# achiever04/face-recognition-platform

Measured on AMD Instinct MI355X. Metric: faces/sec (detect+embed+match) on 1080p @ 100k gallery, higher is better.
Workload: dtype f16; 1 GPU; 32x1080x1920 BGR frames per GPU per step resident in HBM, host results out every step, 2 batches in flight per GPU (one handle = one stream each, used round-robin), forced K=10 faces/frame, 100000-identity fp16 gallery, FRPDet detector fp16 + ArcFace IResNet-100 fp16 (synthetic seeded weights); batch_frames=32, faces_per_frame=10, gallery=100000, streams=1, lanes=2, lane_warmup_steps=20

## Files before the change

### face-recognition-platform_amd/csrc/decode_nms.hip

```cpp
#include <hip/hip_runtime.h>
#include <stdint.h>
#include "frp_internal.h"

namespace frp {

#define NMS_CAP 1024
#define NT 1024

__device__ __forceinline__ unsigned sortable16(unsigned short h) {
    if ((h & 0x7fffu) > 0x7c00u) return 0u;
    return (h & 0x8000u) ? (unsigned)(unsigned short)(~h) : (unsigned)(h | 0x8000u);
}
__device__ __forceinline__ bool is_candidate(_Float16 lg, float lt) {
    return lt == -INFINITY ? true : (float)lg >= lt;
}

struct FrameView {
    const _Float16 *h0, *h1, *h2;
    int w0, w1, w2;
    int e0, e1;
};

__device__ __forceinline__ const _Float16* anchor_ptr(const FrameView& fv, int idx, int& level, int& x, int& y) {
    level = idx < fv.e0 ? 0 : (idx < fv.e1 ? 1 : 2);
    const int li = idx - (level == 0 ? 0 : (level == 1 ? fv.e0 : fv.e1));
    const int wl = level == 0 ? fv.w0 : (level == 1 ? fv.w1 : fv.w2);
    const _Float16* base = level == 0 ? fv.h0 : (level == 1 ? fv.h1 : fv.h2);
    const int pos = li >> 1, a = li & 1;
    y = pos / wl;
    x = pos - y * wl;
    return base + (long)pos * 32 + a * 15;
}

__device__ __forceinline__ FrameView frame_view(const DecodeParams& p, int b, int& A) {
    FrameView fv;
    fv.h0 = p.head[0] + (long)b * p.hl[0] * p.wl[0] * 32;
    fv.h1 = p.head[1] + (long)b * p.hl[1] * p.wl[1] * 32;
    fv.h2 = p.head[2] + (long)b * p.hl[2] * p.wl[2] * 32;
    fv.w0 = p.wl[0]; fv.w1 = p.wl[1]; fv.w2 = p.wl[2];
    fv.e0 = p.hl[0] * p.wl[0] * 2;
    fv.e1 = fv.e0 + p.hl[1] * p.wl[1] * 2;
    A = fv.e1 + p.hl[2] * p.wl[2] * 2;
    return fv;
}

__global__ __launch_bounds__(256) void gather_logits_kernel(DecodeParams p) {
    int A;
    const FrameView fv = frame_view(p, blockIdx.y, A);
    const int i = blockIdx.x * 256 + threadIdx.x;
    if (i >= A) return;
    int lv, x, y;
    p.logits[(long)blockIdx.y * A + i] = anchor_ptr(fv, i, lv, x, y)[0];
}

__global__ __launch_bounds__(NT) void decode_nms_kernel(DecodeParams p) {
    __shared__ unsigned long long keys[NMS_CAP];
    __shared__ int hist[4096];
    __shared__ float bx1[NMS_CAP], by1[NMS_CAP], bx2[NMS_CAP], by2[NMS_CAP], barea[NMS_CAP];
    __shared__ unsigned char supp[NMS_CAP];
    __shared__ int s_cnt, s_digit, s_need, s_keepn;
    __shared__ int s_keep[FRP_MAX_FACES_CAP];
    __shared__ int wsum[NT / 64];

    const int b = blockIdx.x;
    const int tid = threadIdx.x;
    int A;
    const FrameView fv = frame_view(p, b, A);
    const float lt = p.logit_thresh;

    if (tid == 0) { s_cnt = 0; s_keepn = 0; }
    __syncthreads();
    const _Float16* dense = p.logits + (long)b * A;
    int local = 0;
    for (int i = tid; i < A; i += NT) local += is_candidate(dense[i], lt) ? 1 : 0;
#pragma unroll
    for (int o = 32; o > 0; o >>= 1) local += __shfl_xor(local, o);
    if ((tid & 63) == 0) atomicAdd(&s_cnt, local);
    __syncthreads();
    const int total = s_cnt;
    __syncthreads();

    unsigned long long T = 0ull;
    if (total > NMS_CAP) {
        unsigned long long prefix = 0ull;
        int need = NMS_CAP;
        for (int pass = 0; pass < 3; ++pass) {
            const int shift = 24 - 12 * pass;
            for (int i = tid; i < 4096; i += NT) hist[i] = 0;
            __syncthreads();
            for (int i = tid; i < A; i += NT) {
                const _Float16 lg = dense[i];
                if (is_candidate(lg, lt)) {
                    const unsigned long long k = ((unsigned long long)sortable16(__builtin_bit_cast(unsigned short, lg)) << 20) |
                                                 (unsigned long long)(0xFFFFF - i);
                    if (pass == 0 || (k >> (shift + 12)) == prefix) atomicAdd(&hist[(int)((k >> shift) & 0xFFF)], 1);
                }
            }
            __syncthreads();
            const int b0 = tid * 4;
            const int h0 = hist[b0], h1 = hist[b0 + 1], h2 = hist[b0 + 2], h3 = hist[b0 + 3];
            const int mine = h0 + h1 + h2 + h3;
            int v = mine;
#pragma unroll
            for (int o = 1; o < 64; o <<= 1) {
                const int n = __shfl_down(v, o);
                if ((tid & 63) + o < 64) v += n;
            }
            if ((tid & 63) == 0) wsum[tid >> 6] = v;
            __syncthreads();
            int above_waves = 0;
            for (int w = (tid >> 6) + 1; w < NT / 64; ++w) above_waves += wsum[w];
            const int suffix_incl = v + above_waves;
            const int above = suffix_incl - mine;
            int c = above;
            if (c < need && need <= c + h3) { s_digit = b0 + 3; s_need = need - c; }
            c += h3;
            if (c < need && need <= c + h2) { s_digit = b0 + 2; s_need = need - c; }
            c += h2;
            if (c < need && need <= c + h1) { s_digit = b0 + 1; s_need = need - c; }
            c += h1;
            if (c < need && need <= c + h0) { s_digit = b0; s_need = need - c; }
            __syncthreads();
            prefix = (prefix << 12) | (unsigned long long)s_digit;
            need = s_need;
            __syncthreads();
        }
        T = prefix;
    }

    if (tid == 0) s_cnt = 0;
    for (int i = tid; i < NMS_CAP; i += NT) { keys[i] = 0ull; supp[i] = 0; }
    __syncthreads();
    for (int i = tid; i < A; i += NT) {
        const _Float16 lg = dense[i];
        if (is_candidate(lg, lt)) {
            const unsigned long long k = ((unsigned long long)sortable16(__builtin_bit_cast(unsigned short, lg)) << 20) |
                                         (unsigned long long)(0xFFFFF - i);
            if (k >= T) {
                const int s = atomicAdd(&s_cnt, 1);
                if (s < NMS_CAP) keys[s] = k | (1ull << 40);
            }
        }
    }
    __syncthreads();
    const int n = s_cnt < NMS_CAP ? s_cnt : NMS_CAP;

    for (int k2 = 2; k2 <= NMS_CAP; k2 <<= 1) {
        for (int j = k2 >> 1; j > 0; j >>= 1) {
            const int i = tid;
            const int ixj = i ^ j;
            if (ixj > i) {
                const unsigned long long a = keys[i], c = keys[ixj];
                const bool desc = (i & k2) == 0;
                if (desc ? (a < c) : (a > c)) { keys[i] = c; keys[ixj] = a; }
            }
            __syncthreads();
        }
    }

    if (tid < n) {
        const int idx = 0xFFFFF - (int)(keys[tid] & 0xFFFFF);
        int lv, x, y;
        const _Float16* q = anchor_ptr(fv, idx, lv, x, y);
        const float s = (float)(8 << lv);
        const float cx = (float)(x * (8 << lv)), cy = (float)(y * (8 << lv));
        const float x1 = cx - (float)q[1] * s, y1 = cy - (float)q[2] * s;
        const float x2 = cx + (float)q[3] * s, y2 = cy + (float)q[4] * s;
        bx1[tid] = x1; by1[tid] = y1; bx2[tid] = x2; by2[tid] = y2;
        barea[tid] = (x2 - x1 + 1.0f) * (y2 - y1 + 1.0f);
    }
    __syncthreads();

    const int K = p.max_faces;
    for (int i = 0; i < n; ++i) {
        if (supp[i]) continue;
        if (tid == 0) s_keep[s_keepn] = i;
        const int kept = s_keepn + 1;
        if (kept >= K) { __syncthreads(); if (tid == 0) s_keepn = kept; __syncthreads(); break; }
        const float ix1 = bx1[i], iy1 = by1[i], ix2 = bx2[i], iy2 = by2[i], ia = barea[i];
        for (int j = i + 1 + tid; j < n; j += NT) {
            const float xx1 = fmaxf(ix1, bx1[j]), yy1 = fmaxf(iy1, by1[j]);
            const float xx2 = fminf(ix2, bx2[j]), yy2 = fminf(iy2, by2[j]);
            const float w = fmaxf(0.0f, xx2 - xx1 + 1.0f), h = fmaxf(0.0f, yy2 - yy1 + 1.0f);
            const float inter = w * h;
            const float ovr = inter / ((ia + barea[j]) - inter);
            if (ovr > p.nms_iou) supp[j] = 1;
        }
        __syncthreads();
        if (tid == 0) s_keepn = kept;
        __syncthreads();
    }
    __syncthreads();
    const int kept = s_keepn;

    if (tid < K) {
        float* ob = p.boxes + ((long)b * K + tid) * 4;
        float* ok = p.kps + ((long)b * K + tid) * 10;
        if (tid < kept) {
            const int c = s_keep[tid];
            const int idx = 0xFFFFF - (int)(keys[c] & 0xFFFFF);
            int lv, x, y;
            const _Float16* q = anchor_ptr(fv, idx, lv, x, y);
            const float s = (float)(8 << lv);
            const float cx = (float)(x * (8 << lv)), cy = (float)(y * (8 << lv));
            ob[0] = bx1[c]; ob[1] = by1[c]; ob[2] = bx2[c]; ob[3] = by2[c];
#pragma unroll
            for (int t = 0; t < 5; ++t) {
                ok[2 * t] = cx + (float)q[5 + 2 * t] * s;
                ok[2 * t + 1] = cy + (float)q[6 + 2 * t] * s;
            }
            p.scores[(long)b * K + tid] = 1.0f / (1.0f + expf(-(float)q[0]));
            if (p.anchor) p.anchor[(long)b * K + tid] = idx;
        } else {
            ob[0] = ob[1] = ob[2] = ob[3] = 0.f;
            for (int t = 0; t < 10; ++t) ok[t] = 0.f;
            p.scores[(long)b * K + tid] = 0.f;
            if (p.anchor) p.anchor[(long)b * K + tid] = -1;
        }
    }
    if (tid == 0) p.counts[b] = kept;
}

__global__ __launch_bounds__(256) void resize_u8_kernel(const uint8_t* __restrict__ src, int B, int H, int W,
                                                        uint8_t* __restrict__ dst, int Hs, int Ws, float ry, float rx) {
    const long total = (long)B * Hs * Ws;
    for (long i = (long)blockIdx.x * blockDim.x + threadIdx.x; i < total; i += (long)gridDim.x * blockDim.x) {
        const int x = (int)(i % Ws);
        const long r = i / Ws;
        const int y = (int)(r % Hs);
        const int b = (int)(r / Hs);
        float sy = ((float)y + 0.5f) * ry - 0.5f, sx = ((float)x + 0.5f) * rx - 0.5f;
        sy = fminf(fmaxf(sy, 0.0f), (float)(H - 1));
        sx = fminf(fmaxf(sx, 0.0f), (float)(W - 1));
        const int y0 = (int)sy, x0 = (int)sx;
        const int y1 = y0 + 1 < H ? y0 + 1 : H - 1, x1 = x0 + 1 < W ? x0 + 1 : W - 1;
        const float fy = sy - (float)y0, fx = sx - (float)x0;
        const uint8_t* p00 = src + (((long)b * H + y0) * W + x0) * 3;
        const uint8_t* p01 = src + (((long)b * H + y0) * W + x1) * 3;
        const uint8_t* p10 = src + (((long)b * H + y1) * W + x0) * 3;
        const uint8_t* p11 = src + (((long)b * H + y1) * W + x1) * 3;
        uint8_t* o = dst + i * 3;
#pragma unroll
        for (int c = 0; c < 3; ++c) {
            const float top = (float)p00[c] * (1.0f - fx) + (float)p01[c] * fx;
            const float bot = (float)p10[c] * (1.0f - fx) + (float)p11[c] * fx;
            const float v = top * (1.0f - fy) + bot * fy;
            o[c] = (uint8_t)fminf(fmaxf(floorf(v + 0.5f), 0.0f), 255.0f);
        }
    }
}

hipError_t launch_resize_u8(const uint8_t* src, int B, int H, int W, uint8_t* dst, int Hs, int Ws, hipStream_t stream) {
    if (!src || !dst || B <= 0 || H <= 0 || W <= 0 || Hs <= 0 || Ws <= 0) return hipErrorInvalidValue;
    const long total = (long)B * Hs * Ws;
    const int grid = (int)((total + 255) / 256 < 16384 ? (total + 255) / 256 : 16384);
    hipLaunchKernelGGL(resize_u8_kernel, dim3(grid), dim3(256), 0, stream, src, B, H, W, dst, Hs, Ws,
                       (float)H / (float)Hs, (float)W / (float)Ws);
    return hipGetLastError();
}

hipError_t launch_decode_nms(const DecodeParams& p, hipStream_t stream) {
    if (p.B <= 0 || p.max_faces <= 0 || p.max_faces > FRP_MAX_FACES_CAP) return hipErrorInvalidValue;
    long A = 0;
    for (int l = 0; l < 3; ++l) {
        if (!p.head[l] || p.hl[l] <= 0 || p.wl[l] <= 0) return hipErrorInvalidValue;
        A += (long)p.hl[l] * p.wl[l] * 2;
    }
    if (A > 0xFFFFF) return hipErrorInvalidValue;
    if (!p.boxes || !p.kps || !p.scores || !p.counts || !p.logits) return hipErrorInvalidValue;
    hipLaunchKernelGGL(gather_logits_kernel, dim3((unsigned)((A + 255) / 256), p.B), dim3(256), 0, stream, p);
    hipError_t e = hipGetLastError();
    if (e != hipSuccess) return e;
    hipLaunchKernelGGL(decode_nms_kernel, dim3(p.B), dim3(NT), 0, stream, p);
    return hipGetLastError();
}

}
```

### face-recognition-platform_amd/csrc/frp_api.cpp

```cpp
#include <hip/hip_runtime.h>

#include <algorithm>
#include <cmath>
#include <cstdio>
#include <cstdlib>
#include <cstring>
#include <mutex>
#include <string>
#include <vector>

#include "frp.h"
#include "frp_blob.h"
#include "frp_internal.h"
#include "frp_handle.h"

using namespace frp;

#define FRP_WINO_MIN_FACES 128
Switches frp::read_switches() {
    auto set = [](const char* n) { return getenv(n) ? 1 : 0; };
    const char *sm = getenv("FRP_SMALL_M"), *wm = getenv("FRP_WINO_MIN_FACES");
    Switches s{};
    s.small_m = !sm ? 0 : (sm[0] == '0' ? -1 : 1);
    s.wino_min_faces = wm ? atoi(wm) : FRP_WINO_MIN_FACES;
    s.s2 = set("FRP_S2"); s.host_count = set("FRP_HOST_COUNT"); s.match_v1 = set("FRP_MATCH_V1");
    s.no_fused_stem12 = set("FRP_NO_FUSED_STEM12"); s.no_fused_stem = set("FRP_NO_FUSED_STEM");
    s.no_emb_stem = set("FRP_NO_EMB_STEM"); s.no_stem_fuse = set("FRP_NO_STEM_FUSE");
    s.no_wino = set("FRP_NO_WINO"); s.no_kconcat = set("FRP_NO_KCONCAT");
    s.no_block_fuse = set("FRP_NO_BLOCK_FUSE"); s.block_fuse_all = set("FRP_BLOCK_FUSE_ALL");
    return s;
}

const ProcessSwitches& frp::process_switches() {
    static const ProcessSwitches s = [] {
        const char* jh = getenv("FRP_JPEG_DEVICE_HUFFMAN");
        const char* js = getenv("FRP_JPEG_SELFSYNC");
        return ProcessSwitches{getenv("FRP_NO_GRAPH") != nullptr, getenv("FRP_C64_ALL") != nullptr, !jh ? 0 : (jh[0] == '0' ? -1 : 1), js && js[0] != '0'};
    }();
    return s;
}

namespace {

float logit_threshold(float t) {
    if (!(t > 0.f)) return -INFINITY;
    if (t >= 1.f) return INFINITY;
    return (float)std::log((double)t / (1.0 - (double)t));
}

bool det_size_ok(int Hs, int Ws) { return Hs > 0 && Ws > 0 && Hs <= 16384 && Ws <= 16384; }

int select_det_source(frp_handle* h, int Hs, int Ws) {
    if (h->rB <= 0) return fail(h, FRP_ERR_INVALID, "no resident frames (call frp_upload_frames)");
    if (!det_size_ok(Hs, Ws)) return fail(h, FRP_ERR_INVALID, "bad detector size");
    if (Hs == h->rH && Ws == h->rW) {
        h->det_scaled = false;
    } else {
        FRPCHK(ensure(h, h->scaled, (size_t)h->rB * Hs * Ws * 3));
        hipError_t e = launch_resize_u8((const uint8_t*)h->frames.p, h->rB, h->rH, h->rW, (uint8_t*)h->scaled.p, Hs, Ws, h->stream);
        if (e != hipSuccess) return fail(h, FRP_ERR_HIP, std::string("resize: ") + hipGetErrorString(e));
        h->det_scaled = true;
    }
    h->dH = Hs; h->dW = Ws;
    h->canvas_h = round_up(Hs, 32);
    h->canvas_w = round_up(Ws, 32);
    return FRP_OK;
}

int ensure_results(frp_handle* h, int B, int K) {
    const size_t s = (size_t)B * K;
    FRPCHK(ensure(h, h->boxes, s * 4 * 4));
    FRPCHK(ensure(h, h->kps, s * 10 * 4));
    FRPCHK(ensure(h, h->scores, s * 4));
    FRPCHK(ensure(h, h->anchor, s * 4));
    FRPCHK(ensure(h, h->counts, (size_t)B * 4));
    FRPCHK(ensure(h, h->face_slot, s * 4));
    FRPCHK(ensure(h, h->nfaces, 16));
    return FRP_OK;
}

struct DetOut {
    float *boxes, *kps, *scores;
    int32_t* counts;
};

int run_decode(frp_handle* h, const void* const head[3], const int dims[3][2], int B, int K, float det_thresh, float nms_iou, uint32_t flags,
               const DetOut* out = nullptr) {
    DecodeParams dp{};
    size_t anchors = 0;
    for (int l = 0; l < 3; ++l) {
        dp.head[l] = (const _Float16*)head[l];
        dp.hl[l] = dims[l][0];
        dp.wl[l] = dims[l][1];
        anchors += (size_t)dp.hl[l] * dp.wl[l] * 2;
    }
    dp.B = B;
    dp.max_faces = K;
    const bool forced = flags & FRP_FLAG_FORCED_K;
    dp.logit_thresh = forced ? -INFINITY : logit_threshold(det_thresh);
    dp.nms_iou = forced ? 2.0f : nms_iou;
    if (out) {
        dp.boxes = out->boxes; dp.kps = out->kps; dp.scores = out->scores; dp.counts = out->counts;
    } else {
        dp.boxes = (float*)h->boxes.p; dp.kps = (float*)h->kps.p; dp.scores = (float*)h->scores.p;
        dp.anchor = (int32_t*)h->anchor.p; dp.counts = (int32_t*)h->counts.p;
    }
    FRPCHK(ensure(h, h->dense_logits, (size_t)B * anchors * 2));
    dp.logits = (_Float16*)h->dense_logits.p;
    const hipError_t e = launch_decode_nms(dp, h->stream);
    if (e != hipSuccess) return fail(h, FRP_ERR_HIP, std::string("decode_nms: ") + hipGetErrorString(e));
    return FRP_OK;
}

int compact_faces(frp_handle* h, int B, int K) {
    hipError_t e = launch_compact_faces((const int32_t*)h->counts.p, B, K, (int32_t*)h->face_slot.p, (int32_t*)h->nfaces.p, h->stream);
    if (e != hipSuccess) return fail(h, FRP_ERR_HIP, std::string("compact_faces: ") + hipGetErrorString(e));
    return FRP_OK;
}

StemParams stem_params(const frp_handle* h, uint32_t flags) {
    StemParams sp{};
    sp.frames = h->det_scaled ? (const uint8_t*)h->scaled.p : (const uint8_t*)h->frames.p;
    sp.B = h->rB; sp.H = h->dH; sp.W = h->dW;
    sp.row_stride = (long)h->dW * 3; sp.frame_stride = (long)h->dH * h->dW * 3;
    sp.Hc = h->canvas_h; sp.Wc = h->canvas_w; sp.Ho = sp.Hc / 2; sp.Wo = sp.Wc / 2;
    sp.rgb_in = (flags & FRP_FLAG_RGB) ? 1 : 0;
    return sp;
}

bool det_wino(const frp_handle* h) {
    return (long)h->rB * (h->canvas_h / 8) * (h->canvas_w / 8) >= 2L * 240 * (h->n_cu > 0 ? h->n_cu : 256);
}

int run_detect(frp_handle* h, const Switches& sw, int K, float det_thresh, float nms_iou, uint32_t flags, const DetOut* out = nullptr) {
    if (!h->have_weights) return fail(h, FRP_ERR_NO_WEIGHTS, "no weights loaded");
    if (h->rB <= 0) return fail(h, FRP_ERR_INVALID, "no resident frames (call frp_upload_frames)");
    if (K <= 0 || K > FRP_MAX_FACES_CAP) return fail(h, FRP_ERR_INVALID, "max_faces out of range");
    const int B = h->rB, Hc = h->canvas_h, Wc = h->canvas_w;
    const bool fused = h->det.det_stem && !sw.no_fused_stem;
    FRPCHK(plan_net(h, h->det, B, Hc, Wc, fused));
    if (!out) FRPCHK(ensure_results(h, B, K));
    const StemParams sp = stem_params(h, flags);
    if (!fused) {
        hipError_t e = launch_preprocess(sp.frames, B, sp.H, sp.W, sp.row_stride, sp.frame_stride, (_Float16*)h->det.bufs[h->det.in_buf].p, Hc, Wc,
                                         sp.rgb_in, h->stream);
        if (e != hipSuccess) return fail(h, FRP_ERR_HIP, std::string("preprocess: ") + hipGetErrorString(e));
    }
    rec(h, EV_PRE);
    FRPCHK(run_net(h, sw, h->det, B, Hc, Wc, &h->ctr.det_conv_flops, &h->ctr.det_conv_launches, fused ? &sp : nullptr, nullptr, det_wino(h)));
    rec(h, EV_DET);
    const void* head[3];
    int dims[3][2];
    for (int l = 0; l < 3; ++l) {
        const int bi = (int)h->hdr.det_head_buf[l];
        head[l] = h->det.bufs[bi].p;
        dims[l][0] = h->det.dims[bi].h;
        dims[l][1] = h->det.dims[bi].w;
        if (h->det.dims[bi].c != 32) return fail(h, FRP_ERR_BLOB, "detector head must have 32 channels");
    }
    FRPCHK(run_decode(h, head, dims, B, K, det_thresh, nms_iou, flags, out));
    if (!out && !(flags & FRP_FLAG_TRACK)) FRPCHK(compact_faces(h, B, K));
    rec(h, EV_DEC);
    return FRP_OK;
}

int run_embed(frp_handle* h, const Switches& sw, int n, const int32_t* n_dev = nullptr, int family_count = -1) {
    if (n <= 0) return FRP_OK;
    if (family_count < 0) family_count = n;
    FcSplitK fc;
    FRPCHK(run_net(h, sw, h->emb, n, FRP_CHIP, FRP_CHIP, &h->ctr.emb_conv_flops, &h->ctr.emb_conv_launches, nullptr, n_dev,
                   family_count >= sw.wino_min_faces, &fc));
    rec(h, EV_EMB);
    FRPCHK(stage_queries(h, n));
    hipError_t e = launch_l2norm((float*)h->emb.bufs[h->hdr.emb_out_buf].p, (_Float16*)h->m.q16.p, n, FRP_EMB_DIM, h->stream,
                                 fc.ksplit != 0 && fc.ksplit != 1 ? (const float*)h->splitk_ws.p : nullptr, fc.ksplit, fc.bias, n_dev, fc.ktot,
                                 h->n_cu);
    if (e != hipSuccess) return fail(h, FRP_ERR_HIP, std::string("l2norm: ") + hipGetErrorString(e));
    rec(h, EV_L2);
    return FRP_OK;
}

int run_align(frp_handle* h, int K, int n, const int32_t* n_dev, uint32_t flags, void* chips) {
    AlignParams ap{};
    ap.frames = (const uint8_t*)h->frames.p;
    ap.B = h->rB; ap.H = h->rH; ap.W = h->rW;
    ap.row_stride = (long)h->rW * 3;
    ap.frame_stride = (long)h->rH * h->rW * 3;
    ap.kps = (const float*)h->kps.p;
    if (K > 0) {
        ap.counts = (const int32_t*)h->counts.p;
        ap.face_slot = (const int32_t*)h->face_slot.p;
// ... 230 lines not shown
        h->pin_stage = nullptr;
        h->pin_cap = 0;
    }
    const size_t want = std::max<size_t>(bytes, 1 << 20);
    void* p = nullptr;
    if (hipHostMalloc(&p, want, hipHostMallocDefault) != hipSuccess) return fail(h, FRP_ERR_OOM, "hipHostMalloc (result staging) failed");
    h->pin_stage = (unsigned char*)p;
    h->pin_cap = want;
    return FRP_OK;
}

int frp::settle_count(frp_handle* h, bool stream_is_idle) {
    Pass& p = h->pass;
    if (p.nfaces >= 0) return FRP_OK;
    if (!stream_is_idle) HIPCHK(h, hipStreamSynchronize(h->stream));
    int n = *h->h_nfaces;
    const bool corrupt = n < 0 || n > p.cap;
    if (corrupt) n = 0;
    p.nfaces = n;
    h->ctr.faces += n;
    if (p.pend_cap > 0) {
        h->ctr.emb_conv_flops += p.pend_flops * n / p.pend_cap - p.pend_flops;
        h->ctr.f8_conv_flops += p.pend_f8flops * n / p.pend_cap - p.pend_f8flops;
    }
    p.pend_cap = 0;
    p.pend_flops = p.pend_f8flops = 0.0;
    return corrupt ? fail(h, FRP_ERR_HIP, "corrupt face count") : FRP_OK;
}

void frp::settle_events(frp_handle* h, bool stream_is_idle) {
    if (!h->ev_pending) return;
    h->ev_pending = false;
    if (!stream_is_idle && hipStreamSynchronize(h->stream) != hipSuccess) return;
    accumulate_events(h, false);
}

extern "C" {

const char* frp_version(void) { return "frp 0.1 (gfx950)"; }

int frp_create(int device, const frp_config* cfg, frp_handle** out) {
    if (!out) return FRP_ERR_INVALID;
    *out = nullptr;
    int ndev = 0;
    if (hipGetDeviceCount(&ndev) != hipSuccess || ndev <= 0) return FRP_ERR_HIP;
    if (device < 0 || device >= ndev) return FRP_ERR_INVALID;
    frp_handle* h = new (std::nothrow) frp_handle();
    if (!h) return FRP_ERR_OOM;
    h->device = device;
    h->cfg.struct_size = sizeof(frp_config);
    h->cfg.max_batch = 32; h->cfg.max_faces = 10; h->cfg.max_h = 1080; h->cfg.max_w = 1920; h->cfg.profile = 0;
    if (cfg) {
        if (cfg->struct_size != (int32_t)sizeof(frp_config)) { delete h; return FRP_ERR_INVALID; }
        if (cfg->max_batch > 0) h->cfg.max_batch = cfg->max_batch;
        if (cfg->max_faces > 0) h->cfg.max_faces = std::min<int>(cfg->max_faces, FRP_MAX_FACES_CAP);
        if (cfg->max_h > 0) h->cfg.max_h = cfg->max_h;
        if (cfg->max_w > 0) h->cfg.max_w = cfg->max_w;
        h->cfg.profile = cfg->profile ? 1 : 0;
    }
    bool ok = hipSetDevice(device) == hipSuccess && hipStreamCreateWithFlags(&h->stream, hipStreamNonBlocking) == hipSuccess;
    for (int i = 0; ok && i < EV_COUNT; ++i) ok = hipEventCreate(&h->ev[i]) == hipSuccess;
    ok = ok && hipHostMalloc((void**)&h->h_nfaces, 64, hipHostMallocDefault) == hipSuccess;
    if (ok) {
        hipDeviceProp_t prop;
        if (hipGetDeviceProperties(&prop, device) == hipSuccess && prop.multiProcessorCount > 0) h->n_cu = prop.multiProcessorCount;
    }
    ok = ok && init_ingest(h);
    if (!ok) { frp_destroy(h); return FRP_ERR_HIP; }
    h->ctr.struct_size = sizeof(frp_counters);
    *out = h;
    return FRP_OK;
}

void frp_destroy(frp_handle* h) {
    if (!h) return;
    (void)hipSetDevice(h->device);
    if (h->stream) (void)hipStreamSynchronize(h->stream);
    if (h->in.copy_stream) (void)hipStreamSynchronize(h->in.copy_stream);
    dist_shutdown(h);
    drop_graphs(h);
    for (DevBuf& b : h->det.bufs) release(b);
    for (DevBuf& b : h->emb.bufs) release(b);
    DevBuf* all[] = {&h->wdata, &h->frames, &h->boxes, &h->kps, &h->scores, &h->counts, &h->anchor, &h->face_slot, &h->nfaces,
                     &h->pyr_boxes, &h->pyr_kps, &h->pyr_scores, &h->pyr_counts, &h->m.q16, &h->m.part_cos, &h->m.part_idx, &h->m.best_cos, &h->m.best_idx, &h->m.hit_cnt, &h->m.hit_idx, &h->m.hit_cos, &h->m.q_groups, &h->m.frame_groups_dev, &h->g_groups_dev, &h->scratch, &h->splitk_ws, &h->dense_logits, &h->scaled, &h->gallery,
                     &h->g_reserved, &h->gx, &h->gx_q, &h->gx_out, &h->det_hashes, &h->quality_in, &h->quality_out,
                     &h->jenc_in, &h->jenc_coef, &h->jenc_work, &h->jenc_bits, &h->jenc_out};
    for (DevBuf* b : all) release(*b);
    for (int i = 0; i < EV_COUNT; ++i) if (h->ev[i]) (void)hipEventDestroy(h->ev[i]);
    if (h->m.frame_groups_ev) (void)hipEventDestroy(h->m.frame_groups_ev);
    release_tracks(h);
    if (h->h_nfaces) (void)hipHostFree(h->h_nfaces);
    if (h->pin_stage) (void)hipHostFree(h->pin_stage);
    release_ingest(h);
    if (h->stream) (void)hipStreamDestroy(h->stream);
    delete h;
}

const char* frp_last_error(const frp_handle* h) { return h ? h->err.c_str() : "null handle"; }

int frp_load_weights(frp_handle* h, const void* blob, size_t bytes) {
    if (!h) return FRP_ERR_INVALID;
    Guard g(h);
    h->have_weights = false;
    ++h->alloc_epoch;
    if (!blob || bytes < sizeof(frp_blob_header)) return fail(h, FRP_ERR_BLOB, "blob too small");
    frp_blob_header hd;
    memcpy(&hd, blob, sizeof(hd));
    if (memcmp(hd.magic, FRP_BLOB_MAGIC, 8) != 0 || hd.version != FRP_BLOB_VERSION || hd.header_bytes != sizeof(frp_blob_header))
        return fail(h, FRP_ERR_BLOB, "bad magic/version");
    if (hd.data_offset > bytes || hd.data_bytes > bytes - hd.data_offset) return fail(h, FRP_ERR_BLOB, "data section out of range");
    if (hd.emb_dim != FRP_EMB_DIM || hd.emb_size != FRP_CHIP || hd.det_in_ch != 8 || hd.emb_in_ch != 8 || hd.det_num_anchors != 2)
        return fail(h, FRP_ERR_BLOB, "unsupported network geometry");
    std::vector<unsigned char> image;
    FRPCHK(load_program(h, hd, (const unsigned char*)blob, bytes, read_switches(), image));
    FRPCHK(ensure(h, h->wdata, image.size()));
    HIPCHK(h, hipMemcpyAsync(h->wdata.p, image.data(), image.size(), hipMemcpyHostToDevice, h->stream));
    HIPCHK(h, hipStreamSynchronize(h->stream));
    h->hdr = hd;
    h->have_weights = true;
    return FRP_OK;
}

int64_t frp_debug_graph_replays(frp_handle* h) {
    if (!h) return -1;
    Guard g(h);
    return h->graph_replays;
}

int frp_process_resident(frp_handle* h, int32_t max_faces, float det_thresh, float nms_iou, uint32_t flags) {
    if (!h) return FRP_ERR_INVALID;
    Guard g(h);
    rec(h, EV_H2D);
    FRPCHK(run_pipeline(h, max_faces, det_thresh, nms_iou, flags));
    h->ev_pending = h->cfg.profile != 0;
    h->ctr.calls += 1;
    return FRP_OK;
}

int frp_process_pyramid(frp_handle* h, int32_t n_scales, const int32_t* det_hw, int32_t per_scale, int32_t max_faces, float det_thresh,
                        float nms_iou, uint32_t flags) {
    if (!h) return FRP_ERR_INVALID;
    Guard g(h);
    if (flags & FRP_FLAG_TRACK) return fail(h, FRP_ERR_INVALID, "process_pyramid: FRP_FLAG_TRACK is not supported under a cross-scale merge");
    FRPCHK(check_match_flags(h, flags, h->rB));
    if (!h->have_weights) return fail(h, FRP_ERR_INVALID, "process_pyramid: no weights loaded");
    if (h->rB <= 0) return fail(h, FRP_ERR_INVALID, "process_pyramid: no resident frames (call frp_upload_frames)");
    if (n_scales < 1 || n_scales > FRP_PYRAMID_MAX_SCALES || !det_hw) return fail(h, FRP_ERR_INVALID, "process_pyramid: 1 to 4 scales");
    if (per_scale < 1 || per_scale > FRP_MAX_FACES_CAP) return fail(h, FRP_ERR_INVALID, "process_pyramid: per_scale out of range");
    if (max_faces < 1 || max_faces > FRP_MAX_FACES_CAP) return fail(h, FRP_ERR_INVALID, "process_pyramid: max_faces out of range");
    if (n_scales * per_scale > FRP_PYRAMID_MAX_CAND)
        return fail(h, FRP_ERR_INVALID, "process_pyramid: more than 512 candidates per frame (n_scales x per_scale)");
    for (int s = 0; s < n_scales; ++s)
        if (!det_size_ok(det_hw[2 * s], det_hw[2 * s + 1])) return fail(h, FRP_ERR_INVALID, "process_pyramid: bad detector size");
    if (flags & FRP_FLAG_FORCED_K)
        return fail(h, FRP_ERR_INVALID, "process_pyramid: FRP_FLAG_FORCED_K has no meaning under a cross-scale merge");
    rec(h, EV_H2D);
    FRPCHK(run_pyramid(h, n_scales, det_hw, per_scale, max_faces, det_thresh, nms_iou, flags));
    h->ev_pending = h->cfg.profile != 0;
    h->ctr.calls += 1;
    return FRP_OK;
}

int frp_synchronize(frp_handle* h) {
    if (!h) return FRP_ERR_INVALID;
    Guard g(h, false);
    HIPCHK(h, hipStreamSynchronize(h->stream));
    FRPCHK(settle_count(h, true));
// ... 262 lines not shown
```

### face-recognition-platform_amd/csrc/frp_handle.h

```cpp
#pragma once
#include <hip/hip_runtime.h>

#include <algorithm>
#include <mutex>
#include <string>
#include <utility>
#include <vector>

#include "frp.h"
#include "frp_blob.h"
#include "frp_internal.h"
#include "net_program.h"

enum { EV_START = 0, EV_H2D, EV_PRE, EV_DET, EV_DEC, EV_ALIGN, EV_EMB, EV_L2, EV_MATCH, EV_D2H, EV_COUNT };

struct Ingest {
    frp::DevBuf frames_next;
    int nB = 0, nH = 0, nW = 0;
    bool next_valid = false;
    hipStream_t copy_stream = nullptr;
    hipEvent_t ev_next_ready = nullptr, ev_next_free = nullptr;
    std::vector<void*> pinned;
    void* jpeg_pin[2] = {nullptr, nullptr};
    size_t jpeg_pin_cap[2] = {0, 0};
// ... 3 lines not shown
    frp::DevBuf jpeg_scan, jpeg_err;
    bool jpeg_selfsync = false;
    int jpeg_selfsync_bytes = 0;
    int64_t ctr_jpeg_selfsync_batches = 0;
    frp::DevBuf jpeg_ss;
    hipEvent_t ev_jpeg_h2d[2] = {nullptr, nullptr};
    bool jpeg_h2d_pending[2] = {false, false};
    frp::DevBuf yuv_stage, yuv_tab;
    void* yuv_pin = nullptr;
    int yuv_turn = 0;
    hipEvent_t ev_yuv[2] = {nullptr, nullptr};
    bool yuv_pending[2] = {false, false};
};

struct Matcher {
    frp::DevBuf q16;
    frp::DevBuf part_cos, part_idx, best_cos, best_idx;
    float within_min_cos = 0.f;
    int within_cap = 0;
    frp::DevBuf hit_cnt, hit_idx, hit_cos;
    frp::DevBuf q_groups;
    std::vector<uint32_t> frame_groups;
    frp::DevBuf frame_groups_dev;
    bool frame_groups_dirty = false, frame_groups_copying = false;
    hipEvent_t frame_groups_ev = nullptr;
};

struct Tracks {
    int max_streams = 0;
    float iou_min = 0.f;
    int refresh = 0, max_missed = 0;
    bool stale = false;
    frp::DevBuf hdr, meta, tab_emb, plan, totals;
    std::vector<int32_t> streams, present;
    frp::DevBuf streams_dev;
    bool streams_dirty = false, streams_copying = false;
    hipEvent_t streams_ev = nullptr;
    int B = 0, K = 0;
    frp::DevBuf slot_i32, slot_emb, slot_idx, slot_cos;
};

struct Pass {
    int B = 0, K = 0;
    int nfaces = 0;
    int cap = 0;
    bool matched = false;
    int within_cap = 0;
    bool within_lists = false;
    bool q16_of_pass = false;
    bool groups = false;
    bool tracked = false, track_matched = false;
    int pend_cap = 0;
    double pend_flops = 0.0, pend_f8flops = 0.0;
};

struct frp_handle {
    int device = 0;
    hipStream_t stream = nullptr;
    std::mutex mu;
    std::string err;
    frp_config cfg{};
    bool have_weights = false;
    frp_blob_header hdr{};
    frp::DevBuf wdata;
    frp::Net det, emb;
    frp::DevBuf frames;
    int rB = 0, rH = 0, rW = 0;
    int n_cu = 256;
    Ingest in;
    frp::DevBuf scaled;
    int dH = 0, dW = 0;
    bool det_scaled = false;
    int canvas_h = 0, canvas_w = 0;
    int det_op_limit = -1;
    std::vector<frp::NetGraph> graphs;
    std::vector<std::string> graph_seen, graph_bad;
    uint64_t alloc_epoch = 1;
    int64_t graph_replays = 0;
    void* comm = nullptr;
    int dist_rank = 0, dist_world = 0;
    frp::DevBuf det_hashes;
    bool det_hash_on = false;
    frp::DevBuf boxes, kps, scores, counts, anchor, face_slot, nfaces, scratch, splitk_ws, dense_logits;
    frp::DevBuf pyr_boxes, pyr_kps, pyr_scores, pyr_counts;
    Matcher m;
    Pass pass;
    Tracks trk;
    bool ev_pending = false;
    frp::DevBuf quality_in, quality_out;
    frp::DevBuf jenc_in, jenc_coef, jenc_work, jenc_bits, jenc_out;
    int32_t* h_nfaces = nullptr;
    unsigned char* pin_stage = nullptr;
    size_t pin_cap = 0;
    frp::DevBuf gallery;
    int64_t g_rows = 0;
    frp::DevBuf g_reserved;
    bool g_exact = false;
    frp::DevBuf gx, gx_q, gx_out;
    std::vector<uint32_t> g_groups;
    frp::DevBuf g_groups_dev;
    bool g_groups_dev_ok = false;
    hipEvent_t ev[EV_COUNT]{};
    frp_counters ctr{};
};

namespace frp {

inline int fail(frp_handle* h, int code, const std::string& msg) {
    if (h) h->err = msg;
    return code;
}

#define HIPCHK(h, expr)                                                                              \
    do {                                                                                             \
        hipError_t _e = (expr);                                                                      \
        if (_e != hipSuccess)                                                                        \
            return fail(h, FRP_ERR_HIP, std::string(#expr) + ": " + hipGetErrorString(_e));          \
    } while (0)

#define FRPCHK(expr)                 \
    do {                             \
        int _r = (expr);             \
        if (_r != FRP_OK) return _r; \
    } while (0)

inline int ensure(frp_handle* h, DevBuf& b, size_t bytes) {
    if (bytes <= b.cap && b.p) return FRP_OK;
    if (b.p) {
        HIPCHK(h, hipStreamSynchronize(h->stream));
        HIPCHK(h, hipFree(b.p));
        b.p = nullptr;
        b.cap = 0;
    }
    const size_t want = std::max<size_t>(bytes, 256);
    ++h->alloc_epoch;
    hipError_t e = hipMalloc(&b.p, want);
    if (e != hipSuccess) {
        b.p = nullptr;
        return fail(h, FRP_ERR_OOM, std::string("hipMalloc(") + std::to_string(want) + "): " + hipGetErrorString(e));
    }
    b.cap = want;
    return FRP_OK;
}

inline void release(DevBuf& b) {
    if (b.p) (void)hipFree(b.p);
    b.p = nullptr;
    b.cap = 0;
}

#define FRP_LOCAL __attribute__((visibility("hidden")))

class FRP_LOCAL ScopedBuf {
    DevBuf b;
    friend int ensure(frp_handle* h, ScopedBuf& s, size_t bytes) { return ensure(h, s.b, bytes); }

public:
    ScopedBuf() = default;
    ScopedBuf(const ScopedBuf&) = delete;
    ScopedBuf& operator=(const ScopedBuf&) = delete;
    ~ScopedBuf() { release(b); }
    const DevBuf* operator->() const { return &b; }
    DevBuf take() { return std::exchange(b, DevBuf()); }
};

FRP_LOCAL void settle_events(frp_handle* h, bool stream_is_idle);
// ... 27 lines not shown
```

### face-recognition-platform_amd/csrc/frp_internal.h

```cpp
#pragma once
#include <hip/hip_runtime.h>
#include <stdint.h>
#include <type_traits>

#define FRP_ACT_NONE 0
#define FRP_ACT_RELU 1
#define FRP_ACT_PRELU 2
#define FRP_FLAG_BORDER_BIAS 1
#define FRP_FLAG_OUT_F32 2
#define FRP_FLAG_RES_UP2 4
#define FRP_FLAG_FLATTEN 8
#define FRP_FLAG_F8 32
#define FRP_FLAG_OUT_FP8 64
#define FRP_CHIP_PIX (112 * 112)
#ifndef FRP_MAX_FACES_CAP
#define FRP_MAX_FACES_CAP 128
#endif

#include "jpeg_host.h"
#include "jpeg_selfsync.h"

namespace frp {

struct Switches {
// ... 142 lines not shown
    const int per_img = strips * segs;
    it.n = item / per_img;
    const int r = item - it.n * per_img, seg = r / strips;
    it.ys = seg * seg_rows;
    it.ye = it.ys + seg_rows < H ? it.ys + seg_rows : H;
    it.x0 = (r - seg * strips) * BLOCK64_STRIP_W;
    it.K = (it.ye - it.ys + 2 + 3) >> 2;
    return it;
}
#define BLOCK64_HALO_UP 2
#define BLOCK64_HALO_DOWN 7
__host__ __device__ inline int block64_first_in_row(const Block64Item& it) { return it.ys - 6 + 4; }
__host__ __device__ inline int block64_last_in_row(const Block64Item& it) { return it.ys - 6 + 4 * (it.K + 1) + 3; }
int conv3x3_block64_variant(int act1, int flags1, bool slope1, int act2, int flags2);
bool conv3x3_block64_plan(int N, int H, int W, int n_cu, Block64Plan* plan);
bool conv3x3_block64_pays(const Block64Plan& plan);
hipError_t launch_conv3x3_block64(const Block64Params& p, hipStream_t stream);
bool conv3x3_s2_eligible(const ConvParams& p);
hipError_t launch_conv3x3_s2(const ConvParams& p, hipStream_t stream);
int conv3x3_wino_form(const ConvParams& p);
bool conv3x3_wino_shape_ok(int W, int Cin, int ksize, int stride);
bool conv3x3_wino_call_ok(int N, int H, int W, int Cin, int Cout, int ksize, int stride, int n_cu, bool has_res, int dbg);
bool conv3x3_wino_wide_pays(int N, int H, int W, int Cin, int Cout, int n_cu, bool has_res);
#ifdef FRP_LAB
bool conv3x3_wino_lab_shape_ok(int W, int Cin, int ksize, int stride);
#endif
size_t conv3x3_wino_image_bytes(int Cin, int Cout);
hipError_t launch_conv3x3_wino(const ConvParams& p, int form, hipStream_t stream);

hipError_t launch_preprocess(const uint8_t* bgr, int B, int H, int W, long row_stride, long frame_stride,
                             _Float16* out, int Hc, int Wc, int rgb_in, hipStream_t stream);

struct StemParams {
    const uint8_t* frames;
    int B, H, W;
    long row_stride, frame_stride;
    int Hc, Wc;
    int Ho, Wo;
    int rgb_in;
    const _Float16* w;
    const float* bias;
    _Float16* out;
};
hipError_t launch_stem_u8(const StemParams& p, hipStream_t stream);

struct Stem12Params {
    const uint8_t* frames;
    int B, H, W;
    long row_stride, frame_stride;
    int Hc, Wc;
    int Ho1, Wo1;
    int Ho2, Wo2;
    int rgb_in;
    const _Float16* w1;
    const float* bias1;
    const _Float16* w2;
    const float* bias2;
    _Float16* out;
};
hipError_t launch_stem12_u8(const Stem12Params& p, hipStream_t stream);

struct EmbStemParams {
    const _Float16* x;
    int M, H, W;
    const _Float16* w;
    const float* bias;
    const float* slope;
    _Float16* out;
    const int32_t* n_dev;
};
hipError_t launch_emb_stem(const EmbStemParams& p, hipStream_t stream);

struct DecodeParams {
    const _Float16* head[3];
    int hl[3], wl[3];
    int B, max_faces;
    float logit_thresh, nms_iou;
    float* boxes;
    float* kps;
    float* scores;
    int32_t* anchor;
    int32_t* counts;
    _Float16* logits;
};
hipError_t launch_decode_nms(const DecodeParams& p, hipStream_t stream);

#define FRP_PYRAMID_MAX_SCALES 4
#define FRP_PYRAMID_MAX_CAND 512
struct PyramidMergeParams {
    const float* boxes;
    const float* kps;
    const float* scores;
    const int32_t* counts;
    int S, B, P, max_faces;
    int frame_h, frame_w;
    int det_h[FRP_PYRAMID_MAX_SCALES], det_w[FRP_PYRAMID_MAX_SCALES];
    float nms_iou;
    float* out_boxes;
    float* out_kps;
    float* out_scores;
    int32_t* out_anchor;
    int32_t* out_counts;
    float rx[FRP_PYRAMID_MAX_SCALES], ry[FRP_PYRAMID_MAX_SCALES];
};
hipError_t launch_pyramid_merge(PyramidMergeParams p, hipStream_t stream);

struct JpegParams {
    const int16_t* coef;
    const uint16_t* qtab;
    uint8_t* planes;
    uint8_t* frames;
    int B, W, H, components;
    int bx[3], by[3];
    int blocks_per_image;
    long plane_off[3], plane_img;
    int hs, vs;
    int cw, ch;
};
hipError_t launch_jpeg_decode(const JpegParams& p, hipStream_t stream);

struct YuvCoef { int yoff, cy, cvr, cvg, cug, cub, rnd, sh; };
struct YuvParams {
    const uint8_t* const* tab;
    uint8_t* frames;
    int B, W, H;
    int64_t y_pitch, c_pitch;
    int ush;
    YuvCoef k;
};
hipError_t launch_yuv_to_bgr(const YuvParams& p, bool semi_planar, bool fast, hipStream_t stream);

struct JpegHuffParams {
    const uint8_t* scan;
    const uint32_t* int_off;
    const JpegHuffTableDev* tables;
    int16_t* coef;
    int32_t* err;
    long coef_per_image;
    int B, n_int, ri;
    int mcus_y;
    JssGeom g;
};
hipError_t launch_jpeg_huffman(const JpegHuffParams& p, hipStream_t stream);

struct JpegSelfsyncParams {
    const uint8_t* scan;
    const uint32_t* img;
    const JpegHuffTableDev* tables;
    JssState* entry;
    JssState* exit_;
    JssState* wgx;
    uint32_t* cnt;
    uint32_t* base;
    int32_t* rounds;
    int32_t* stats;
    int16_t* coef;
    long coef_per_image;
    int B, S;
    uint32_t max_sub;
    uint32_t n_wg_all;
    JssGeom g;
};
hipError_t launch_jpeg_selfsync_round(const JpegSelfsyncParams& p, int k, hipStream_t stream);
hipError_t launch_jpeg_selfsync_finish(const JpegSelfsyncParams& p, hipStream_t stream);

hipError_t launch_tensor_hash(const void* src, size_t bytes, unsigned long long* slot, hipStream_t stream);
hipError_t launch_resize_u8(const uint8_t* src, int B, int H, int W, uint8_t* dst, int Hs, int Ws, hipStream_t stream);
// ... 184 lines not shown
```

Before: 28600 faces/s.

## Build score histogram during logit gather to replace per-frame radix select passes

The gather kernel now processes 1024 anchors per workgroup, writes the logits to a padded dense buffer, and accumulates an 11-bit score histogram per frame in global memory. The decode/NMS kernel reads that histogram to find the cutoff bin in one step, then makes a single vectorized pass over the logits. It collects keys above the bin directly and ranks the cut-bin keys in LDS, instead of a count pass plus three radix-histogram passes over all anchors. A fallback to the old 3-pass select remains for when the cut bin overflows its buffer. The cost is global atomics in the gather, a persistent histogram buffer that the kernel must re-zero each step, and a quadratic rank over up to 2048 cut-bin keys.

Result: no change. 28710 faces/s, median of 6 (+0.4%).

```diff
diff --git a/face-recognition-platform_amd/csrc/decode_nms.hip b/face-recognition-platform_amd/csrc/decode_nms.hip
--- a/face-recognition-platform_amd/csrc/decode_nms.hip
+++ b/face-recognition-platform_amd/csrc/decode_nms.hip
@@ -1,11 +1,16 @@
 #include <hip/hip_runtime.h>
 #include <stdint.h>
 #include "frp_internal.h"
+#include "decode_select_host.h"
 
 namespace frp {
 
 #define NMS_CAP 1024
 #define NT 1024
+#define CUT_CAP 2048
+#define GATHER_PER_WG 1024
+
+typedef _Float16 half8 __attribute__((ext_vector_type(8)));
 
 __device__ __forceinline__ unsigned sortable16(unsigned short h) {
     if ((h & 0x7fffu) > 0x7c00u) return 0u;
@@ -13,6 +18,9 @@
 }
 __device__ __forceinline__ bool is_candidate(_Float16 lg, float lt) {
     return lt == -INFINITY ? true : (float)lg >= lt;
+}
+__device__ __forceinline__ unsigned long long anchor_key(_Float16 lg, int i) {
+    return ((unsigned long long)sortable16(__builtin_bit_cast(unsigned short, lg)) << 20) | (unsigned long long)(0xFFFFF - i);
 }
 
 struct FrameView {
@@ -43,47 +51,99 @@
     A = fv.e1 + p.hl[2] * p.wl[2] * 2;
     return fv;
 }
+__device__ __forceinline__ long dense_stride(int A) { return (long)((A + 7) & ~7); }
 
 __global__ __launch_bounds__(256) void gather_logits_kernel(DecodeParams p) {
+    __shared__ int lh[DECODE_HIST_BINS];
     int A;
-    const FrameView fv = frame_view(p, blockIdx.y, A);
-    const int i = blockIdx.x * 256 + threadIdx.x;
-    if (i >= A) return;
-    int lv, x, y;
-    p.logits[(long)blockIdx.y * A + i] = anchor_ptr(fv, i, lv, x, y)[0];
+    const int b = blockIdx.y, tid = threadIdx.x;
+    const FrameView fv = frame_view(p, b, A);
+    for (int i = tid; i < DECODE_HIST_BINS; i += 256) lh[i] = 0;
+    __syncthreads();
+    _Float16* dense = p.logits + (long)b * dense_stride(A);
+    _Float16 lg[GATHER_PER_WG / 256];
+#pragma unroll
+    for (int j = 0; j < GATHER_PER_WG / 256; ++j) {
+        const int i = blockIdx.x * GATHER_PER_WG + j * 256 + tid;
+        int lv, x, y;
+        lg[j] = i < A ? anchor_ptr(fv, i, lv, x, y)[0] : (_Float16)0.f;
+    }
+#pragma unroll
+    for (int j = 0; j < GATHER_PER_WG / 256; ++j) {
+        const int i = blockIdx.x * GATHER_PER_WG + j * 256 + tid;
+        if (i < A) {
+            dense[i] = lg[j];
+            if (is_candidate(lg[j], p.logit_thresh)) atomicAdd(&lh[decode_hist_bin(sortable16(__builtin_bit_cast(unsigned short, lg[j])))], 1);
+        }
+    }
+    __syncthreads();
+    int32_t* row = p.hist + (long)b * DECODE_HIST_BINS;
+    for (int i = tid; i < DECODE_HIST_BINS; i += 256) {
+        const int c = lh[i];
+        if (c) atomicAdd(&row[i], c);
+    }
 }
 
 __global__ __launch_bounds__(NT) void decode_nms_kernel(DecodeParams p) {
     __shared__ unsigned long long keys[NMS_CAP];
-    __shared__ int hist[4096];
+    __shared__ unsigned long long cutk[CUT_CAP];
     __shared__ float bx1[NMS_CAP], by1[NMS_CAP], bx2[NMS_CAP], by2[NMS_CAP], barea[NMS_CAP];
     __shared__ unsigned char supp[NMS_CAP];
-    __shared__ int s_cnt, s_digit, s_need, s_keepn;
+    __shared__ int s_cnt, s_cutc, s_total, s_digit, s_need, s_keepn;
     __shared__ int s_keep[FRP_MAX_FACES_CAP];
     __shared__ int wsum[NT / 64];
+    int* hist = reinterpret_cast<int*>(cutk);
+    static_assert(CUT_CAP * 8 == 4096 * 4, "the side buffer and the radix histogram share their LDS");
+    static_assert(DECODE_HIST_BINS == 2 * NT, "two histogram bins per thread");
 
     const int b = blockIdx.x;
     const int tid = threadIdx.x;
     int A;
     const FrameView fv = frame_view(p, b, A);
     const float lt = p.logit_thresh;
-
-    if (tid == 0) { s_cnt = 0; s_keepn = 0; }
-    __syncthreads();
-    const _Float16* dense = p.logits + (long)b * A;
-    int local = 0;
-    for (int i = tid; i < A; i += NT) local += is_candidate(dense[i], lt) ? 1 : 0;
-#pragma unroll
-    for (int o = 32; o > 0; o >>= 1) local += __shfl_xor(local, o);
-    if ((tid & 63) == 0) atomicAdd(&s_cnt, local);
-    __syncthreads();
-    const int total = s_cnt;
-    __syncthreads();
-
-    unsigned long long T = 0ull;
-    if (total > NMS_CAP) {
+    const _Float16* dense = p.logits + (long)b * dense_stride(A);
+
+    if (tid == 0) { s_cnt = 0; s_cutc = 0; s_keepn = 0; s_digit = -1; s_need = 0; }
+    for (int i = tid; i < NMS_CAP; i += NT) { keys[i] = 0ull; supp[i] = 0; }
+    int total, cut = -1, need = 0;
+    bool fallback;
+    {
+        int2* row = reinterpret_cast<int2*>(p.hist + (long)b * DECODE_HIST_BINS);
+        const int2 hv = row[tid];
+        row[tid] = make_int2(0, 0);
+        const int h2[2] = {hv.x, hv.y};
+        const int mine = hv.x + hv.y;
+        int v = mine;
+#pragma unroll
+        for (int o = 1; o < 64; o <<= 1) {
+            const int n = __shfl_down(v, o);
+            if ((tid & 63) + o < 64) v += n;
+        }
+        if ((tid & 63) == 0) wsum[tid >> 6] = v;
+        __syncthreads();
+        int above_waves = 0;
+        for (int w = (tid >> 6) + 1; w < NT / 64; ++w) above_waves += wsum[w];
+        const int suffix_incl = v + above_waves;
+        if (tid == 0) s_total = suffix_incl;
+        int bin, above_bin;
+        if (decode_cut_bin(h2, 2 * tid, 2, suffix_incl - mine, NMS_CAP, &bin, &above_bin)) {
+            s_digit = bin;
+            s_need = NMS_CAP - above_bin;
+            s_cutc = h2[bin - 2 * tid];
+        }
+        __syncthreads();
+        total = s_total;
+        if (total > NMS_CAP) { cut = s_digit; need = s_need; }
+        fallback = total > NMS_CAP && s_cutc > CUT_CAP;
+        __syncthreads();
+        if (tid == 0) s_cutc = 0;
+    }
+
+    int n;
+    if (fallback) {
+        unsigned long long T = 0ull;
         unsigned long long prefix = 0ull;
-        int need = NMS_CAP;
+        need = NMS_CAP;
         for (int pass = 0; pass < 3; ++pass) {
             const int shift = 24 - 12 * pass;
             for (int i = tid; i < 4096; i += NT) hist[i] = 0;
@@ -91,59 +151,80 @@
             for (int i = tid; i < A; i += NT) {
                 const _Float16 lg = dense[i];
                 if (is_candidate(lg, lt)) {
-                    const unsigned long long k = ((unsigned long long)sortable16(__builtin_bit_cast(unsigned short, lg)) << 20) |
-                                                 (unsigned long long)(0xFFFFF - i);
+                    const unsigned long long k = anchor_key(lg, i);
                     if (pass == 0 || (k >> (shift + 12)) == prefix) atomicAdd(&hist[(int)((k >> shift) & 0xFFF)], 1);
                 }
             }
             __syncthreads();
             const int b0 = tid * 4;
-            const int h0 = hist[b0], h1 = hist[b0 + 1], h2 = hist[b0 + 2], h3 = hist[b0 + 3];
-            const int mine = h0 + h1 + h2 + h3;
+            const int h4[4] = {hist[b0], hist[b0 + 1], hist[b0 + 2], hist[b0 + 3]};
+            const int mine = h4[0] + h4[1] + h4[2] + h4[3];
             int v = mine;
 #pragma unroll
             for (int o = 1; o < 64; o <<= 1) {
-                const int n = __shfl_down(v, o);
-                if ((tid & 63) + o < 64) v += n;
+                const int nn = __shfl_down(v, o);
+                if ((tid & 63) + o < 64) v += nn;
             }
             if ((tid & 63) == 0) wsum[tid >> 6] = v;
             __syncthreads();
             int above_waves = 0;
             for (int w = (tid >> 6) + 1; w < NT / 64; ++w) above_waves += wsum[w];
-            const int suffix_incl = v + above_waves;
-            const int above = suffix_incl - mine;
-            int c = above;
-            if (c < need && need <= c + h3) { s_digit = b0 + 3; s_need = need - c; }
-            c += h3;
-            if (c < need && need <= c + h2) { s_digit = b0 + 2; s_need = need - c; }
-            c += h2;
-            if (c < need && need <= c + h1) { s_digit = b0 + 1; s_need = need - c; }
-            c += h1;
-            if (c < need && need <= c + h0) { s_digit = b0; s_need = need - c; }
+            int bin, above_bin;
+            if (decode_cut_bin(h4, b0, 4, v + above_waves - mine, need, &bin, &above_bin)) { s_digit = bin; s_need = need - above_bin; }
             __syncthreads();
             prefix = (prefix << 12) | (unsigned long long)s_digit;
             need = s_need;
             __syncthreads();
         }
         T = prefix;
-    }
-
-    if (tid == 0) s_cnt = 0;
-    for (int i = tid; i < NMS_CAP; i += NT) { keys[i] = 0ull; supp[i] = 0; }
-    __syncthreads();
-    for (int i = tid; i < A; i += NT) {
-        const _Float16 lg = dense[i];
-        if (is_candidate(lg, lt)) {
-            const unsigned long long k = ((unsigned long long)sortable16(__builtin_bit_cast(unsigned short, lg)) << 20) |
-                                         (unsigned long long)(0xFFFFF - i);
-            if (k >= T) {
-                const int s = atomicAdd(&s_cnt, 1);
-                if (s < NMS_CAP) keys[s] = k | (1ull << 40);
-            }
-        }
-    }
-    __syncthreads();
-    const int n = s_cnt < NMS_CAP ? s_cnt : NMS_CAP;
+        for (int i = tid; i < A; i += NT) {
+            const _Float16 lg = dense[i];
+            if (is_candidate(lg, lt)) {
+                const unsigned long long k = anchor_key(lg, i);
+                if (k >= T) {
+                    const int s = atomicAdd(&s_cnt, 1);
+                    if (s < NMS_CAP) keys[s] = k | (1ull << 40);
+                }
+            }
+        }
+        __syncthreads();
+        n = s_cnt < NMS_CAP ? s_cnt : NMS_CAP;
+    } else {
+        __syncthreads();
+        const half8* dv = reinterpret_cast<const half8*>(dense);
+        const int nvec = (A + 7) >> 3;
+        for (int vi = tid; vi < nvec; vi += NT) {
+            const half8 v8 = dv[vi];
+#pragma unroll
+            for (int e = 0; e < 8; ++e) {
+                const int i = vi * 8 + e;
+                const _Float16 lg = v8[e];
+                if (i < A && is_candidate(lg, lt)) {
+                    const unsigned long long k = anchor_key(lg, i);
+                    const int bin = decode_hist_bin((unsigned)(k >> 20));
+                    if (bin > cut) {
+                        const int s = atomicAdd(&s_cnt, 1);
+                        if (s < NMS_CAP) keys[s] = k | (1ull << 40);
+                    } else if (bin == cut) {
+                        const int c = atomicAdd(&s_cutc, 1);
+                        if (c < CUT_CAP) cutk[c] = k;
+                    }
+                }
+            }
+        }
+        __syncthreads();
+        const int nab = s_cnt < NMS_CAP ? s_cnt : NMS_CAP;
+        const int nc = s_cutc < CUT_CAP ? s_cutc : CUT_CAP;
+        for (int c = tid; c < nc; c += NT) {
+            const unsigned long long k = cutk[c];
+            int rank = 0;
+            for (int j = 0; j < nc; ++j) rank += cutk[j] > k ? 1 : 0;
+            if (rank < need && nab + rank < NMS_CAP) keys[nab + rank] = k | (1ull << 40);
+        }
+        __syncthreads();
+        const int from_cut = need < nc ? need : nc;
+        n = nab + from_cut < NMS_CAP ? nab + from_cut : NMS_CAP;
+    }
 
     for (int k2 = 2; k2 <= NMS_CAP; k2 <<= 1) {
         for (int j = k2 >> 1; j > 0; j >>= 1) {
@@ -259,6 +340,8 @@
     return hipGetLastError();
 }
 
+size_t decode_hist_bytes(size_t B) { return B * DECODE_HIST_BINS * sizeof(int32_t); }
+
 hipError_t launch_decode_nms(const DecodeParams& p, hipStream_t stream) {
     if (p.B <= 0 || p.max_faces <= 0 || p.max_faces > FRP_MAX_FACES_CAP) return hipErrorInvalidValue;
     long A = 0;
@@ -267,8 +350,8 @@
         A += (long)p.hl[l] * p.wl[l] * 2;
     }
     if (A > 0xFFFFF) return hipErrorInvalidValue;
-    if (!p.boxes || !p.kps || !p.scores || !p.counts || !p.logits) return hipErrorInvalidValue;
-    hipLaunchKernelGGL(gather_logits_kernel, dim3((unsigned)((A + 255) / 256), p.B), dim3(256), 0, stream, p);
+    if (!p.boxes || !p.kps || !p.scores || !p.counts || !p.logits || !p.hist) return hipErrorInvalidValue;
+    hipLaunchKernelGGL(gather_logits_kernel, dim3((unsigned)((A + GATHER_PER_WG - 1) / GATHER_PER_WG), p.B), dim3(256), 0, stream, p);
     hipError_t e = hipGetLastError();
     if (e != hipSuccess) return e;
     hipLaunchKernelGGL(decode_nms_kernel, dim3(p.B), dim3(NT), 0, stream, p);
diff --git a/face-recognition-platform_amd/csrc/decode_select_host.h b/face-recognition-platform_amd/csrc/decode_select_host.h
--- /dev/null
+++ b/face-recognition-platform_amd/csrc/decode_select_host.h
@@ -0,0 +1,21 @@
+#pragma once
+#include <hip/hip_runtime.h>
+#include <stdint.h>
+
+namespace frp {
+
+#define DECODE_HIST_BITS 11
+#define DECODE_HIST_BINS (1 << DECODE_HIST_BITS)
+__host__ __device__ __forceinline__ int decode_hist_bin(unsigned sortable16) { return (int)(sortable16 >> (16 - DECODE_HIST_BITS)); }
+
+__host__ __device__ __forceinline__ bool decode_cut_bin(const int* hist, int lo, int n, int above, int need, int* bin, int* above_bin) {
+    int c = above;
+    for (int b = lo + n - 1; b >= lo; --b) {
+        const int hb = hist[b - lo];
+        if (c < need && need <= c + hb) { *bin = b; *above_bin = c; return true; }
+        c += hb;
+    }
+    return false;
+}
+
+}
diff --git a/face-recognition-platform_amd/csrc/frp_api.cpp b/face-recognition-platform_amd/csrc/frp_api.cpp
--- a/face-recognition-platform_amd/csrc/frp_api.cpp
+++ b/face-recognition-platform_amd/csrc/frp_api.cpp
@@ -105,8 +105,12 @@
         dp.boxes = (float*)h->boxes.p; dp.kps = (float*)h->kps.p; dp.scores = (float*)h->scores.p;
         dp.anchor = (int32_t*)h->anchor.p; dp.counts = (int32_t*)h->counts.p;
     }
-    FRPCHK(ensure(h, h->dense_logits, (size_t)B * anchors * 2));
+    FRPCHK(ensure(h, h->dense_logits, decode_logits_bytes((size_t)B, anchors)));
     dp.logits = (_Float16*)h->dense_logits.p;
+    const void* const hist_before = h->decode_hist.p;
+    FRPCHK(ensure(h, h->decode_hist, decode_hist_bytes((size_t)B)));
+    if (h->decode_hist.p != hist_before) HIPCHK(h, hipMemsetAsync(h->decode_hist.p, 0, h->decode_hist.cap, h->stream));
+    dp.hist = (int32_t*)h->decode_hist.p;
     const hipError_t e = launch_decode_nms(dp, h->stream);
     if (e != hipSuccess) return fail(h, FRP_ERR_HIP, std::string("decode_nms: ") + hipGetErrorString(e));
     return FRP_OK;
@@ -503,7 +507,7 @@
     for (DevBuf& b : h->det.bufs) release(b);
     for (DevBuf& b : h->emb.bufs) release(b);
     DevBuf* all[] = {&h->wdata, &h->frames, &h->boxes, &h->kps, &h->scores, &h->counts, &h->anchor, &h->face_slot, &h->nfaces,
-                     &h->pyr_boxes, &h->pyr_kps, &h->pyr_scores, &h->pyr_counts, &h->m.q16, &h->m.part_cos, &h->m.part_idx, &h->m.best_cos, &h->m.best_idx, &h->m.hit_cnt, &h->m.hit_idx, &h->m.hit_cos, &h->m.q_groups, &h->m.frame_groups_dev, &h->g_groups_dev, &h->scratch, &h->splitk_ws, &h->dense_logits, &h->scaled, &h->gallery,
+                     &h->pyr_boxes, &h->pyr_kps, &h->pyr_scores, &h->pyr_counts, &h->m.q16, &h->m.part_cos, &h->m.part_idx, &h->m.best_cos, &h->m.best_idx, &h->m.hit_cnt, &h->m.hit_idx, &h->m.hit_cos, &h->m.q_groups, &h->m.frame_groups_dev, &h->g_groups_dev, &h->scratch, &h->splitk_ws, &h->dense_logits, &h->decode_hist, &h->scaled, &h->gallery,
                      &h->g_reserved, &h->gx, &h->gx_q, &h->gx_out, &h->det_hashes, &h->quality_in, &h->quality_out,
                      &h->jenc_in, &h->jenc_coef, &h->jenc_work, &h->jenc_bits, &h->jenc_out};
     for (DevBuf* b : all) release(*b);
diff --git a/face-recognition-platform_amd/csrc/frp_handle.h b/face-recognition-platform_amd/csrc/frp_handle.h
--- a/face-recognition-platform_amd/csrc/frp_handle.h
+++ b/face-recognition-platform_amd/csrc/frp_handle.h
@@ -109,6 +109,7 @@
     frp::DevBuf det_hashes;
     bool det_hash_on = false;
     frp::DevBuf boxes, kps, scores, counts, anchor, face_slot, nfaces, scratch, splitk_ws, dense_logits;
+    frp::DevBuf decode_hist;
     frp::DevBuf pyr_boxes, pyr_kps, pyr_scores, pyr_counts;
     Matcher m;
     Pass pass;
diff --git a/face-recognition-platform_amd/csrc/frp_internal.h b/face-recognition-platform_amd/csrc/frp_internal.h
--- a/face-recognition-platform_amd/csrc/frp_internal.h
+++ b/face-recognition-platform_amd/csrc/frp_internal.h
@@ -248,7 +248,10 @@
     int32_t* anchor;
     int32_t* counts;
     _Float16* logits;
-};
+    int32_t* hist;
+};
+inline size_t decode_logits_bytes(size_t B, size_t anchors) { return B * ((anchors + 7) & ~(size_t)7) * 2; }
+size_t decode_hist_bytes(size_t B);
 hipError_t launch_decode_nms(const DecodeParams& p, hipStream_t stream);
 
 #define FRP_PYRAMID_MAX_SCALES 4
```
